# danielzgtg/TTS.cpp

Hardware: AMD Instinct MI355X
Metric: audio-sec/wall-sec (RTF^-1), Parler-TTS-mini v1 Q4_K AR decode + DAC decode (higher is better)
Workload: dtype q4_K weights x q8_K activations (int dot, f32 combine); DAC f16 im2col x f32 weights, f64 accumulate

## Files before the change

### include/tts_hip.h

```cpp
#ifndef TTS_HIP_H
#define TTS_HIP_H

#include <stddef.h>
#include <stdint.h>

#ifdef __cplusplus
extern "C" {
#endif

#define TTS_MAX_DIMS 4
#define TTS_MAX_SRC 4
#define TTS_MAX_OP_PARAMS 16
#define TTS_MAX_NAME 64

enum tts_type {
    TTS_TYPE_F32 = 0,
    TTS_TYPE_F16 = 1,
    TTS_TYPE_Q4_0 = 2,
    TTS_TYPE_Q4_1 = 3,
    TTS_TYPE_Q5_0 = 6,
    TTS_TYPE_Q5_1 = 7,
    TTS_TYPE_Q8_0 = 8,
    TTS_TYPE_Q8_1 = 9,
    TTS_TYPE_Q4_K = 12,
// ... 167 lines not shown
    TTS_HIP_OPT_GEMV_RSPLIT = 17,
    TTS_HIP_OPT_ATTN_PV16 = 15,
    TTS_HIP_OPT_GEMV_PREQUANT = 21,
    TTS_HIP_OPT_GEMV_KRELAY = 22,
    TTS_HIP_OPT_ATTN_KS = 23,
    TTS_HIP_OPT_ATTN_PV8 = 24,
    TTS_HIP_OPT_GEMV_KRELAY_LOOP = 26,
    TTS_HIP_OPT_GEMV_Q80_PRO = 27,
    TTS_HIP_OPT_GEMV_Q80_SLAB = 28,
    TTS_HIP_OPT_GEMV_Q80_RW = 29,
    TTS_HIP_OPT_GEMM_Q8_STAGED = 30,
    TTS_HIP_OPT_GEMV_KR_INKERNEL = 31,
    TTS_HIP_OPT_GEMV_F32_WIDE = 32,
    TTS_HIP_OPT_ATTN_PV_MP = 33,
    TTS_HIP_OPT_GEMM_KR_INKERNEL = 35,
    TTS_HIP_OPT_GEMM_KR_CT2 = 36,
    TTS_HIP_OPT_GEMM_KR_NW = 34,
    TTS_HIP_OPT_GEMV_NW_MIN = 25,
    TTS_HIP_OPT_GEMM_KR_XCD = 38,
    TTS_HIP_OPT_GEMM_KR_CP = 39,
    TTS_HIP_OPT_GEMM_KR_WALK = 40,
    TTS_HIP_OPT_GEMM_PF = 41,
    TTS_HIP_OPT_GEMM_PF_NW = 42,
    TTS_HIP_OPT_ATTN_ONE = 43,
    TTS_HIP_OPT_GEMV_KR_TAIL = 44,
    TTS_HIP_OPT_GEMV_Q50_SLAB = 45,
    TTS_HIP_OPT_GEMV_Q50_RW = 46,
    TTS_HIP_OPT_GEMM_Q5 = 47,
    TTS_HIP_OPT_GEMM_Q5_STAGED = 48,
    TTS_HIP_OPT_GEMV_Q40_SLAB = 49,
    TTS_HIP_OPT_GEMV_Q40_RW = 50,
    TTS_HIP_OPT_GEMM_Q4_0 = 51,
    TTS_HIP_OPT_GEMM_Q4_0_STAGED = 52,
    TTS_HIP_OPT_COALESCE = 37,
};
enum tts_fuse_bits {
    TTS_FUSE_LN = 1, TTS_FUSE_GROUP = 2, TTS_FUSE_KV = 4, TTS_FUSE_EPI = 8, TTS_FUSE_HEADS = 16, TTS_FUSE_ATTN = 32,
    TTS_FUSE_LSTM = 64,
    TTS_FUSE_SNAKE = 128,
    TTS_FUSE_EMBED = 256,
    TTS_FUSE_CONV = 512,
    TTS_FUSE_ADAIN = 1024,
    TTS_FUSE_XATTN = 2048,
    TTS_FUSE_MCPY = 4096,
    TTS_FUSE_CONTREAD = 8192
};
int tts_hip_set_option(tts_hip_backend_t backend, int option, int value);
int tts_hip_attn_decode(tts_hip_backend_t backend, const tts_tensor * q, const tts_tensor * k, const tts_tensor * v,
                        const float * mask, int64_t mbs, float scale, float * out, float * out2, const int64_t * koff,
                        const int64_t * voff, const int64_t * moff, const int32_t * pseq);
int tts_hip_coalesce_stats(int device, int64_t * out, int n);
void tts_hip_coalesce_set_wait(int us);
int tts_hip_coalesce_enable(int on);
#define TTS_HIP_HOOK_FAULT_WEIGHT_SET 1
int tts_hip_test_hook(int hook, int value);
int tts_hip_install_crash_handler(void);
int tts_hip_gemv_stats(tts_hip_backend_t backend, int type, double * ms, int64_t * launches, double * bytes, int reset);
int tts_hip_greedy_step(tts_hip_backend_t backend, const float * logits, int32_t B, int32_t NH, int32_t V, int32_t step,
                        int32_t bos, int32_t eos, int32_t * eos_seen, int32_t * hist, int32_t * next);
typedef struct tts_sampling {
    float temperature;
    float top_p;
    float repetition_penalty;
    int32_t top_k;
    int32_t do_sample;
    int32_t pad_;
// ... 48 lines not shown
```

### tts.cpp_amd/csrc/backend.hip

```cpp
#include <cmath>
#include <atomic>
#include <cstring>
#include <map>
#include <mutex>
#include <thread>

#include "hip_internal.h"
#include <hip/hip_ext.h>

#include <dlfcn.h>
#include <execinfo.h>
#include <fcntl.h>
#include <signal.h>
#include <unistd.h>

using namespace tts;


static void build_gelu_table(uint16_t * t) {
    const float GELU_COEF_A = 0.044715f;
    const float SQRT_2_OVER_PI = 0.79788456080286535587989211986876f;
    for (int i = 0; i < 65536; ++i) {
        const float x = fp16_to_fp32_host((uint16_t)i);
        const float g = 0.5f * x * (1.0f + tanhf(SQRT_2_OVER_PI * x * (1.0f + GELU_COEF_A * x * x)));
// ... 50 lines not shown
    if (hipGetDeviceCount(&n) != hipSuccess) return 0;
    return n;
}

tts_hip_backend_t tts_hip_backend_init(int device) {
    int n = tts_hip_device_count();
    if (device < 0 || device >= n) return nullptr;
    if (hipSetDevice(device) != hipSuccess) return nullptr;
    auto * be = new tts_hip_backend();
    be->device = device;
    TTS_HIP_CHECK(hipStreamCreateWithFlags(&be->stream, hipStreamNonBlocking));
    TTS_HIP_CHECK(hipStreamCreateWithFlags(&be->cap_stream, hipStreamNonBlocking));
    TTS_HIP_CHECK(hipStreamCreateWithFlags(&be->pf_stream, hipStreamNonBlocking));
    TTS_HIP_CHECK(hipEventCreateWithFlags(&be->co_ev, hipEventDisableTiming));
    TTS_HIP_CHECK(hipEventCreateWithFlags(&be->pf_fork, hipEventDisableTiming));
    TTS_HIP_CHECK(hipEventCreateWithFlags(&be->pf_join, hipEventDisableTiming));
    hipDeviceProp_t prop;
    TTS_HIP_CHECK(hipGetDeviceProperties(&prop, device));
    snprintf(be->name, sizeof(be->name), "HIP%d(%s)", device, prop.gcnArchName);
    be->cu_total = prop.multiProcessorCount > 0 ? prop.multiProcessorCount : 256;
    be->cus = be->cu_total;
    TTS_HIP_CHECK(hipMalloc((void **)&be->scratch, kScratchBytes));
    be->scratch_size = kScratchBytes;
    TTS_HIP_CHECK(hipMalloc((void **)&be->shadow, kShadowBytes));
    be->shadow_size = kShadowBytes;
    be->hoist_size = (size_t)8 << 20;
    TTS_HIP_CHECK(hipMalloc(&be->hoist, be->hoist_size));
    TTS_HIP_CHECK(hipMalloc((void **)&be->lstm_buf, kLstmFloats * sizeof(float)));
    TTS_HIP_CHECK(hipMalloc((void **)&be->attn_buf, kAttnFloats * sizeof(float)));
    be->attn_floats = kAttnFloats;
    TTS_HIP_CHECK(hipMalloc((void **)&be->vec_scratch, kVecScratchFloats * sizeof(float)));
    be->conv_stage_floats = (size_t)8 << 20;
    TTS_HIP_CHECK(hipMalloc((void **)&be->conv_stage, be->conv_stage_floats * sizeof(float)));
    be->conv_part_doubles = (size_t)8 << 20;
    TTS_HIP_CHECK(hipMalloc((void **)&be->conv_part, be->conv_part_doubles * sizeof(double)));
    be->lstm_floats = kLstmFloats;
    TTS_HIP_CHECK(hipMalloc((void **)&be->argmax_keys, kArgmaxRows * sizeof(unsigned long long)));
    TTS_HIP_CHECK(hipMalloc((void **)&be->argmax_counts, kArgmaxRows * sizeof(unsigned)));
    TTS_HIP_CHECK(hipMemset(be->argmax_keys, 0, kArgmaxRows * sizeof(unsigned long long)));
    TTS_HIP_CHECK(hipMemset(be->argmax_counts, 0, kArgmaxRows * sizeof(unsigned)));
    TTS_HIP_CHECK(hipHostMalloc((void **)&be->pin, kPinBytes, hipHostMallocDefault));
    be->pin_size = kPinBytes;
    for (auto & e : be->plan_ev) TTS_HIP_CHECK(hipEventCreateWithFlags(&e, hipEventDisableTiming));
    std::vector<uint16_t> tab(65536);
    build_gelu_table(tab.data());
    TTS_HIP_CHECK(hipMalloc((void **)&be->gelu_table, 65536 * sizeof(uint16_t)));
    TTS_HIP_CHECK(hipMemcpy(be->gelu_table, tab.data(), 65536 * sizeof(uint16_t), hipMemcpyHostToDevice));
    return be;
}

void tts_hip_backend_free(tts_hip_backend_t be) {
    if (!be) return;
    tts::coalesce_backend_gone(be);
    hipSetDevice(be->device);
    hipStreamSynchronize(be->stream);
    for (auto & p : be->ev_pending) {
        hipEventDestroy(p.first);
        hipEventDestroy(p.second);
    }
    for (auto e : be->ev_free) hipEventDestroy(e);
    for (auto & r : be->pin_pending) hipEventDestroy(r.ev);
    for (auto e : be->pin_events) hipEventDestroy(e);
    for (auto e : be->plan_ev) hipEventDestroy(e);
    hipHostFree(be->pin);
    if (be->rb_host) hipHostFree(be->rb_host);
    hipFree(be->scratch);
// ... 551 lines not shown
        case TTS_OP_IM2COL:
            return is_f32(n->src[1]) && n->op_params[6] == 0 && (n->type == TTS_TYPE_F16 || n->type == TTS_TYPE_F32);
        case TTS_OP_CONV_TRANSPOSE_1D:
            return is_f32(n->src[0]) && is_f32(n->src[1]) && n->op_params[4] >= 1;
        case TTS_OP_CUMSUM: case TTS_OP_UPSCALE: case TTS_OP_STFT: case TTS_OP_ISTFT: case TTS_OP_MAP_CUSTOM3: case TTS_OP_MAP_CUSTOM2:
            return tts::audio_op_supported(n);
        case TTS_OP_GET_ROWS:
            return n->src[1]->type == TTS_TYPE_I32 &&
                   (n->src[0]->type == TTS_TYPE_F32 || n->src[0]->type == TTS_TYPE_F16 || n->src[0]->type == TTS_TYPE_Q4_K ||
                    n->src[0]->type == TTS_TYPE_Q8_0 || n->src[0]->type == TTS_TYPE_Q5_0 || n->src[0]->type == TTS_TYPE_Q4_0);
        case TTS_OP_MUL_MAT: {
            const tts_tensor * a = n->src[0];
            const tts_tensor * b = n->src[1];
            if (!is_f32(b)) return 0;
            if (a->ne[0] != b->ne[0] || b->ne[2] % a->ne[2] || b->ne[3] % a->ne[3]) return 0;
            if (a->type == TTS_TYPE_F32 || a->type == TTS_TYPE_F16) return 1;
            if (a->type == TTS_TYPE_Q4_K) return a->ne[0] % 256 == 0;
            if (a->type == TTS_TYPE_Q8_0 || a->type == TTS_TYPE_Q5_0 || a->type == TTS_TYPE_Q4_0) return a->ne[0] % 32 == 0;
            return 0;
        }
        default:
            return 0;
    }
}

}

extern "C" int tts_hip_set_option(tts_hip_backend_t be, int option, int value) {
    if (!be) return TTS_STATUS_BAD_ARG;
    switch (option) {
        case TTS_HIP_OPT_FUSION: be->fusion = value; return 0;
        case TTS_HIP_OPT_CONVT_LDS: be->convt_lds = value != 0; return 0;
        case TTS_HIP_OPT_CONV_SPLIT: be->conv_split = value < 0 ? 1 : value; return 0;
        case TTS_HIP_OPT_PROFILE_GEMV: be->profile_gemv = value != 0; return 0;
        case TTS_HIP_OPT_GRAPHS: be->use_graphs = value != 0; return 0;
        case TTS_HIP_OPT_CONV_F32ACC:
            be->conv_f32acc = value == 1;
            be->conv_acc_mode = value == 2 ? 2 : 0;
            return 0;
        case TTS_HIP_OPT_ATTN_SPLIT: be->attn_split_minp = value; return 0;
        case TTS_HIP_OPT_ATTN_FUSED: be->attn_fused_minp = value; return 0;
        case TTS_HIP_OPT_ATTN_PV16: be->attn_pv_uv16 = value != 0; return 0;
        case TTS_HIP_OPT_KV_PREFETCH: be->kv_prefetch_minp = value; return 0;
        case TTS_HIP_OPT_Q4K_TILE_BYTES: be->q4k_tile_bytes = value; return 0;
        case TTS_HIP_OPT_Q4K_DUAL_BYTES: be->q4k_dual_bytes = value; return 0;
        case TTS_HIP_OPT_GEMV_RSPLIT: be->gemv_mf_rsplit = value != 0; return 0;
        case TTS_HIP_OPT_GEMV_PREQUANT: be->gemv_mf_prequant = value != 0; return 0;
        case TTS_HIP_OPT_GEMV_KRELAY: be->gemv_kr = value != 0; return 0;
        case TTS_HIP_OPT_GEMV_KRELAY_LOOP: be->gemv_kr_loop = value != 0; return 0;
        case TTS_HIP_OPT_GEMV_Q80_PRO: be->gemv_q80_pro = value != 0; return 0;
        case TTS_HIP_OPT_GEMV_Q80_SLAB: be->gemv_q80_slab = value != 0; return 0;
        case TTS_HIP_OPT_GEMV_KR_INKERNEL:
            if (value < 0) return TTS_STATUS_BAD_ARG;
            be->gemv_kr_ink = value;
            return 0;
        case TTS_HIP_OPT_GEMM_Q8_STAGED:
            if (value < 0 || value > 2) return TTS_STATUS_BAD_ARG;
            be->gemm_q8_staged = value;
            return 0;
        case TTS_HIP_OPT_GEMV_Q80_RW:
            if (value < 0 || value > 32 || (value & (value - 1))) return TTS_STATUS_BAD_ARG;
            be->gemv_q80_rw = value;
            return 0;
        case TTS_HIP_OPT_GEMV_Q50_SLAB: be->gemv_q50_slab = value != 0; return 0;
        case TTS_HIP_OPT_GEMV_Q50_RW:
            if (value < 0 || value > 32 || (value & (value - 1))) return TTS_STATUS_BAD_ARG;
// ... 167 lines not shown
```

### tts.cpp_amd/csrc/hip_internal.h

```cpp
#pragma once

#include <hip/hip_fp16.h>
#include <hip/hip_runtime.h>

#include <cstdio>
#include <cstdlib>
#include <atomic>
#include <deque>
#include <mutex>
#include <unordered_map>
#include <tuple>
#include <vector>

#include "common.h"

#define TTS_HIP_CHECK(expr)                                                                          \
    do {                                                                                             \
        hipError_t err_ = (expr);                                                                    \
        if (err_ != hipSuccess) {                                                                    \
            fprintf(stderr, "%s:%d: HIP error %s: %s\n", __FILE__, __LINE__, #expr, hipGetErrorString(err_)); \
            abort();                                                                                 \
        }                                                                                            \
    } while (0)

// ... 370 lines not shown
    int gemm_kr_ct2 = 0;
    int64_t gemm_kr_ink = 0;
    int gemv_nw_min = 0;
    int gemv_mf_rsplit = 1;
    int64_t q4k_dual_bytes = 1 << 20;
    void * sample_cand = nullptr;
    size_t sample_cand_size = 0;
    int kv_prefetch_minp = 0;
    int kv_prefetch_blocks = 128;
    hipStream_t pf_stream = nullptr;
    hipEvent_t pf_fork = nullptr, pf_join = nullptr;
    uint8_t * pin = nullptr;
    size_t pin_size = 0, pin_head = 0;
    struct PinRec {
        size_t off, size;
        hipEvent_t ev;
    };
    std::deque<PinRec> pin_pending;
    std::vector<hipEvent_t> pin_events;
    std::mutex pin_mu;
    hipEvent_t plan_ev[2] = {nullptr, nullptr};
    bool plan_ev_pending[2] = {false, false};
    float * lstm_buf = nullptr;
    float * conv_stage = nullptr;
    size_t conv_stage_floats = 0;
    float * vec_scratch = nullptr;
    size_t lstm_floats = 0;
    tts::ActQuant aq;
    int64_t graph_epoch = 0;
    uint16_t * gelu_table = nullptr;
    bool convt_lds = true;
    double * conv_part = nullptr;
    size_t conv_part_doubles = 0;
    int conv_split = 1;
    int fusion = 0x3FFF;
    bool profile_gemv = false;
    double gemv_ms[TTS_TYPE_COUNT] = {0};
    int64_t gemv_launches[TTS_TYPE_COUNT] = {0};
    double gemv_bytes[TTS_TYPE_COUNT] = {0};
    std::vector<std::pair<hipEvent_t, hipEvent_t>> ev_pending;
    std::vector<double> ev_bytes;
    std::vector<int> ev_type;
    std::vector<hipEvent_t> ev_free;
    char * repack_tmp = nullptr;
    size_t repack_tmp_size = 0;
    std::vector<char *> repack_retired;
    float * attn_stage = nullptr;
    size_t attn_stage_size = 0;
    bool use_graphs = false;
    static constexpr int N_GSIG = 4;
    uint64_t gsig[N_GSIG] = {};
    hipGraphExec_t gsig_exec[N_GSIG] = {};
    int gsig_next = 0;
    bool conv_f32acc = false;
    int conv_acc_mode = 0;
    hipStream_t cap_stream = nullptr;
    int64_t graph_updates = 0, graph_instantiations = 0;
    int64_t lstm_chains = 0, lstm_steps = 0;
    int64_t plan_wait_ns = 0;
    int64_t cap_plan_ns = 0, cap_launch_ns = 0, cap_update_ns = 0;
    hipGraphExec_t pexec[2] = {nullptr, nullptr};
    tts_tensor * const * plan_nodes[2] = {nullptr, nullptr};
    int plan_n[2] = {0, 0};
    bool plan_eager[2] = {true, true};
    bool plan_prepared[2] = {false, false};
    tts::BatchCtx * bat = nullptr;
// ... 139 lines not shown
```

### tts.cpp_amd/csrc/k_conv.hip

```cpp
#include "hip_internal.h"

namespace tts {

template <bool F16OUT>
__global__ void k_im2col(TD dst, TD x, int K, int s0, int p0, int d0, int64_t n) {
    const int64_t KW = dst.ne[0];
    const int64_t OL = dst.ne[1];
    const int64_t L = x.ne[0];
    for (int64_t e = (int64_t)blockIdx.x * blockDim.x + threadIdx.x; e < n; e += (int64_t)gridDim.x * blockDim.x) {
        const int64_t kk = e % KW;
        const int64_t ol = (e / KW) % OL;
        const int64_t nn = e / (KW * OL);
        const int64_t ic = kk / K, k = kk % K;
        const int64_t il = ol * s0 + k * d0 - p0;
        float v = 0.f;
        if (il >= 0 && il < L) v = *(const float *)(x.data + il * x.nb[0] + ic * x.nb[1] + nn * x.nb[2]);
        char * o = dst.data + kk * dst.nb[0] + ol * dst.nb[1] + nn * dst.nb[2];
        if (F16OUT) *(__half *)o = __float2half_rn(v);
        else *(float *)o = v;
    }
}

void launch_im2col(tts_hip_backend * be, const tts_tensor * node) {
    const tts_tensor * a = node->src[0];
// ... 186 lines not shown
    if (a->ne[2] * a->ne[3] != 1 || b->ne[2] * b->ne[3] != 1 || node->type != TTS_TYPE_F32) return false;
    const int64_t K = a->ne[0], M = a->ne[1], N = b->ne[1];
    const size_t bes = tts_type_size(b->type);
    if (K % 8 || a->nb[0] != 2 || b->nb[0] != bes || node->nb[0] != 4) return false;
    if (a->nb[1] % 16 || b->nb[1] % 16 || ((uintptr_t)a->data % 16) || ((uintptr_t)b->data % 16)) return false;
    dim3 grid((unsigned)((M + 63) / 64), (unsigned)((N + 63) / 64));
    if (!be->conv_f32acc) {
        const int nz = split_count(be, (int64_t)grid.x * grid.y, K, 256, M * N);
        const int64_t kps = nz > 1 ? (((K + nz - 1) / nz + 31) & ~(int64_t)31) : K;
        const int nzr = nz > 1 ? (int)((K + kps - 1) / kps) : 1;
        double * part = nzr > 1 ? be->conv_part : nullptr;
        grid.z = (unsigned)nzr;
        if (b->type == TTS_TYPE_F16)
            hipLaunchKernelGGL(k_gemm_f16_f64acc<true>, grid, dim3(256), 0, be->stream, (const __half *)a->data, (int64_t)(a->nb[1] / 2), b->data,
                               (int64_t)(b->nb[1] / 2), (float *)node->data, (int64_t)(node->nb[1] / 4), M, N, K, part, kps);
        else
            hipLaunchKernelGGL(k_gemm_f16_f64acc<false>, grid, dim3(256), 0, be->stream, (const __half *)a->data, (int64_t)(a->nb[1] / 2), b->data,
                               (int64_t)(b->nb[1] / 4), (float *)node->data, (int64_t)(node->nb[1] / 4), M, N, K, part, kps);
        TTS_HIP_CHECK(hipGetLastError());
        if (part) launch_split_reduce(be, nzr, M, N, (float *)node->data, (int64_t)(node->nb[1] / 4), nullptr, 0, nullptr, 0);
        return true;
    }
    if (b->type == TTS_TYPE_F16)
        hipLaunchKernelGGL(k_gemm_f16_mfma<true>, grid, dim3(256), 0, be->stream, (const __half *)a->data, (int64_t)(a->nb[1] / 2), b->data,
                           (int64_t)(b->nb[1] / 2), (float *)node->data, (int64_t)(node->nb[1] / 4), M, N, K);
    else
        hipLaunchKernelGGL(k_gemm_f16_mfma<false>, grid, dim3(256), 0, be->stream, (const __half *)a->data, (int64_t)(a->nb[1] / 2), b->data,
                           (int64_t)(b->nb[1] / 4), (float *)node->data, (int64_t)(node->nb[1] / 4), M, N, K);
    TTS_HIP_CHECK(hipGetLastError());
    return true;
}

typedef _Float16 h16x8_t __attribute__((ext_vector_type(8)));
template <bool W16, bool BIAS, bool RES, bool H32 = false>
__global__ __launch_bounds__(256) void k_conv1d_f64(Conv1dArgs a) {
    extern __shared__ float sm[];
    __shared__ int xoff[CONV1D_MAX_R];
    __shared__ int wofs[CONV1D_MAX_R];
    const int lane = threadIdx.x & 63, wave = threadIdx.x >> 6;
    const int c16 = lane & 15, kq = lane >> 4;
    const int64_t ol0 = (int64_t)blockIdx.x * 64;
    const int oc0 = blockIdx.y * 64;
    const int K = a.K, s = a.s, icc = a.icc, xw = a.xw, rs = a.rs;
    const int R = icc * K, Rp = (R + 31) & ~31;
    float * xs = sm;
    float * ws = sm + icc * xw + 1;
    const int zslot = icc * xw;
    for (int r = threadIdx.x; r < Rp; r += 256) {
        const int ic = r / K, k = r - ic * K;
        xoff[r] = r < R ? ic * xw + k * a.d : zslot;
        wofs[r] = r < R ? (int)(k * a.wk + ic * a.wic) : -1;
    }
    if (threadIdx.x == 0) xs[zslot] = 0.f;
    __syncthreads();
    const int wr0 = (wave >> 1) * 32, wc0 = (wave & 1) * 32;
    const bool wave_live = oc0 + wr0 < a.OC && ol0 + wc0 < a.OL;
    f64x4_t acc[2][2] = {};
    const int64_t base = ol0 * s - a.p;
    const int EX = icc * xw, EW = 64 * Rp;
    constexpr int esz = W16 ? 2 : 4;
    const uint32_t OOB = 0x80000000u;
    const auto xr = __builtin_amdgcn_make_buffer_rsrc(a.x.data, 0, a.x_bytes, 0x00020000);
    const auto wr = __builtin_amdgcn_make_buffer_rsrc(const_cast<void *>(a.w), 0, a.w_bytes, 0x00020000);
    uint32_t xrel[CONV1D_XN], wrel[CONV1D_WN];
    int xic[CONV1D_XN], wic[CONV1D_WN];
#pragma unroll
    for (int u = 0; u < CONV1D_XN; ++u) {
        const int e = (int)threadIdx.x + 256 * u;
        const int ic = e / xw, q = e - ic * xw;
        const int64_t pos = base + q;
        const bool ok = e < EX && pos >= 0 && pos < a.L;
        xrel[u] = ok ? (uint32_t)(pos * a.x.nb[0] + (int64_t)ic * a.x.nb[1]) : OOB;
        xic[u] = e < EX ? ic : -1;
    }
#pragma unroll
    for (int u = 0; u < CONV1D_WN; ++u) {
        const int e = (int)threadIdx.x + 256 * u;
        const int oc = e / Rp, r = e - oc * Rp;
        const int wo = e < EW ? wofs[r] : -1;
        const bool ok = wo >= 0 && oc0 + oc < a.OC;
        wrel[u] = ok ? (uint32_t)(((int64_t)(oc0 + oc) * a.woc + wo) * esz) : OOB;
        wic[u] = e < EW ? (r < R ? r / K : icc) : -1;
    }
    float xv[CONV1D_XN], wv[CONV1D_WN];
    auto fetch = [&](int ic0) {
        const int nic = min(icc, (int)(a.IC - ic0));
        const uint32_t xc = (uint32_t)((int64_t)ic0 * a.x.nb[1]);
        const uint32_t wc = (uint32_t)((int64_t)ic0 * a.wic * esz);
#pragma unroll
        for (int u = 0; u < CONV1D_XN; ++u) {
            const uint32_t off = (xrel[u] == OOB || xic[u] >= nic) ? OOB : xrel[u] + xc;
            xv[u] = __builtin_bit_cast(float, __builtin_amdgcn_raw_buffer_load_b32(xr, off, 0, 0));
        }
#pragma unroll
        for (int u = 0; u < CONV1D_WN; ++u) {
            const uint32_t off = (wrel[u] == OOB || wic[u] >= nic) ? OOB : wrel[u] + wc;
            if (W16) wv[u] = __half2float(__builtin_bit_cast(__half, __builtin_amdgcn_raw_buffer_load_b16(wr, off, 0, 0)));
            else wv[u] = __builtin_bit_cast(float, __builtin_amdgcn_raw_buffer_load_b32(wr, off, 0, 0));
        }
    };
    const int ic_lo = a.part ? (int)blockIdx.z * a.ic_per_split : 0;
    const int ic_hi = a.part ? (int)min((int64_t)(ic_lo + a.ic_per_split), a.IC) : (int)a.IC;
    fetch(ic_lo);
    for (int ic0 = ic_lo; ic0 < ic_hi; ic0 += icc) {
#pragma unroll
        for (int u = 0; u < CONV1D_XN; ++u)
            if (xic[u] >= 0) xs[(int)threadIdx.x + 256 * u] = __half2float(__float2half_rn(xv[u]));
#pragma unroll
        for (int u = 0; u < CONV1D_WN; ++u)
            if (wic[u] >= 0) {
                const int e = (int)threadIdx.x + 256 * u;
                const int oc = e / Rp;
                ws[oc * rs + (e - oc * Rp)] = W16 ? wv[u] : __half2float(__float2half_rn(wv[u]));
            }
        __syncthreads();
        if (ic0 + icc < ic_hi) fetch(ic0 + icc);
        if (!wave_live) {
            __syncthreads();
            continue;
        }
        if (H32) {
            for (int r0 = 0; r0 < Rp; r0 += 32) {
                int xo[8];
#pragma unroll
                for (int u = 0; u < 8; ++u) xo[u] = xoff[r0 + 8 * kq + u];
                h16x8_t A[2], B[2];
#pragma unroll
                for (int t = 0; t < 2; ++t)
#pragma unroll
                    for (int u = 0; u < 8; ++u) {
                        const bool z = xo[u] == zslot;
                        A[t][u] = (_Float16)ws[(wr0 + 16 * t + c16) * rs + r0 + 8 * kq + u];
                        B[t][u] = (_Float16)xs[z ? zslot : xo[u] + (wc0 + 16 * t + c16) * s];
                    }
#pragma unroll
                for (int ti = 0; ti < 2; ++ti)
#pragma unroll
                    for (int tj = 0; tj < 2; ++tj) {
                        const f32x4 pr = __builtin_amdgcn_mfma_f32_16x16x32_f16(A[ti], B[tj], f32x4{0.f, 0.f, 0.f, 0.f}, 0, 0, 0);
#pragma unroll
                        for (int e = 0; e < 4; ++e) acc[ti][tj][e] += (double)pr[e];
                    }
            }
        } else
        for (int r0 = 0; r0 < Rp; r0 += 32) {
            int xo[8];
#pragma unroll
            for (int u = 0; u < 8; ++u) xo[u] = xoff[r0 + 4 * u + kq];
            float af[8][2], bf[8][2];
#pragma unroll
            for (int u = 0; u < 8; ++u) {
                const int r = r0 + 4 * u + kq;
                const bool z = xo[u] == zslot;
#pragma unroll
                for (int t = 0; t < 2; ++t) {
                    af[u][t] = ws[(wr0 + 16 * t + c16) * rs + r];
                    bf[u][t] = xs[z ? zslot : xo[u] + (wc0 + 16 * t + c16) * s];
                }
            }
#pragma unroll
            for (int u = 0; u < 8; ++u)
#pragma unroll
                for (int ti = 0; ti < 2; ++ti)
#pragma unroll
                    for (int tj = 0; tj < 2; ++tj)
                        acc[ti][tj] = __builtin_amdgcn_mfma_f64_16x16x4f64((double)af[u][ti], (double)bf[u][tj], acc[ti][tj], 0, 0, 0);
        }
        __syncthreads();
    }
    if (a.part) {
#pragma unroll
        for (int tj = 0; tj < 2; ++tj) {
            const int64_t ol = ol0 + wc0 + 16 * tj + c16;
            if (ol >= a.OL) continue;
#pragma unroll
            for (int ti = 0; ti < 2; ++ti)
#pragma unroll
                for (int e = 0; e < 4; ++e) {
                    const int oc = oc0 + wr0 + 16 * ti + (H32 ? 4 * kq + e : kq + 4 * e);
                    if (oc < a.OC) a.part[((int64_t)blockIdx.z * a.OC + oc) * a.OL + ol] = acc[ti][tj][e];
                }
        }
        return;
    }
    float bv[2][4], rv[2][2][4];
#pragma unroll
    for (int ti = 0; ti < 2; ++ti)
#pragma unroll
        for (int e = 0; e < 4; ++e) {
            const int oc = min(oc0 + wr0 + 16 * ti + (H32 ? 4 * kq + e : kq + 4 * e), (int)a.OC - 1);
            bv[ti][e] = BIAS ? a.bias[(int64_t)oc * a.bcs] : 0.f;
#pragma unroll
            for (int tj = 0; tj < 2; ++tj) {
                const int64_t ol = min(ol0 + wc0 + 16 * tj + c16, a.OL - 1);
                rv[tj][ti][e] = RES ? a.res[ol + (int64_t)oc * a.rcs] : 0.f;
            }
        }
#pragma unroll
    for (int tj = 0; tj < 2; ++tj) {
        const int64_t ol = ol0 + wc0 + 16 * tj + c16;
        if (ol >= a.OL) continue;
#pragma unroll
        for (int ti = 0; ti < 2; ++ti)
#pragma unroll
            for (int e = 0; e < 4; ++e) {
                const int oc = oc0 + wr0 + 16 * ti + (H32 ? 4 * kq + e : kq + 4 * e);
                if (oc >= a.OC) continue;
                float v = (float)acc[ti][tj][e];
                if (BIAS) v = v + bv[ti][e];
                if (RES) v = rv[tj][ti][e] + v;
                a.y[ol + (int64_t)oc * a.ycs] = v;
            }
    }
}

bool conv1d_fused_ok(int64_t IC, int K, int s, int d, size_t * lds) {
    if (K < 1 || K > 64 || s < 1 || d < 1 || IC < 1) return false;
    const int xw = 63 * s + (K - 1) * d + 1;
    const int icc = conv1d_icc(IC, K, xw);
    if (icc < 1) return false;
    const int rs = ((icc * K + 31) & ~31) + 1;
    const size_t bytes = ((size_t)icc * xw + 1 + 64 * (size_t)rs) * 4;
    if (lds) *lds = bytes;
    return bytes <= 64 * 1024;
}

void launch_conv1d_fused(tts_hip_backend * be, Conv1dArgs a) {
    a.xw = 63 * a.s + (a.K - 1) * a.d + 1;
    a.icc = conv1d_icc(a.IC, a.K, a.xw);
    a.rs = ((a.icc * a.K + 31) & ~31) + 1;
    size_t lds = 0;
    if (!conv1d_fused_ok(a.IC, a.K, a.s, a.d, &lds)) {
        fprintf(stderr, "tts_hip: conv1d_fused shape unsupported\n");
        abort();
    }
    dim3 grid((unsigned)((a.OL + 63) / 64), (unsigned)((a.OC + 63) / 64));
    Conv1dArgs e = a;
    const int64_t nchunk = (a.IC + a.icc - 1) / a.icc;
    const int nz = be->conv_acc_mode == 2 ? 1 : split_count(be, (int64_t)grid.x * grid.y, nchunk, 2, a.OL * a.OC);
    if (nz > 1) {
        a.ic_per_split = (int)(((nchunk + nz - 1) / nz) * a.icc);
        grid.z = (unsigned)((a.IC + a.ic_per_split - 1) / a.ic_per_split);
        a.part = be->conv_part;
        a.bias = nullptr;
        a.res = nullptr;
    }
    const int sel = (a.w16 ? 4 : 0) | (a.bias ? 2 : 0) | (a.res ? 1 : 0);
    if (be->conv_acc_mode == 2) switch (sel) {
        case 0: hipLaunchKernelGGL((k_conv1d_f64<false, false, false, true>), grid, dim3(256), lds, be->stream, a); break;
        case 1: hipLaunchKernelGGL((k_conv1d_f64<false, false, true, true>), grid, dim3(256), lds, be->stream, a); break;
        case 2: hipLaunchKernelGGL((k_conv1d_f64<false, true, false, true>), grid, dim3(256), lds, be->stream, a); break;
        case 3: hipLaunchKernelGGL((k_conv1d_f64<false, true, true, true>), grid, dim3(256), lds, be->stream, a); break;
        case 4: hipLaunchKernelGGL((k_conv1d_f64<true, false, false, true>), grid, dim3(256), lds, be->stream, a); break;
        case 5: hipLaunchKernelGGL((k_conv1d_f64<true, false, true, true>), grid, dim3(256), lds, be->stream, a); break;
        case 6: hipLaunchKernelGGL((k_conv1d_f64<true, true, false, true>), grid, dim3(256), lds, be->stream, a); break;
        default: hipLaunchKernelGGL((k_conv1d_f64<true, true, true, true>), grid, dim3(256), lds, be->stream, a); break;
    }
    else switch (sel) {
        case 0: hipLaunchKernelGGL((k_conv1d_f64<false, false, false>), grid, dim3(256), lds, be->stream, a); break;
        case 1: hipLaunchKernelGGL((k_conv1d_f64<false, false, true>), grid, dim3(256), lds, be->stream, a); break;
        case 2: hipLaunchKernelGGL((k_conv1d_f64<false, true, false>), grid, dim3(256), lds, be->stream, a); break;
        case 3: hipLaunchKernelGGL((k_conv1d_f64<false, true, true>), grid, dim3(256), lds, be->stream, a); break;
        case 4: hipLaunchKernelGGL((k_conv1d_f64<true, false, false>), grid, dim3(256), lds, be->stream, a); break;
        case 5: hipLaunchKernelGGL((k_conv1d_f64<true, false, true>), grid, dim3(256), lds, be->stream, a); break;
        case 6: hipLaunchKernelGGL((k_conv1d_f64<true, true, false>), grid, dim3(256), lds, be->stream, a); break;
        default: hipLaunchKernelGGL((k_conv1d_f64<true, true, true>), grid, dim3(256), lds, be->stream, a); break;
    }
    TTS_HIP_CHECK(hipGetLastError());
    if (a.part) launch_split_reduce(be, (int)grid.z, a.OL, a.OC, e.y, e.ycs, e.bias, e.bcs, e.res, e.rcs);
    if (a.copy_dst)
        launch_copy_bytes(be, a.copy_dst, a.y, (size_t)a.OL * (size_t)a.OC * 4);
}

__global__ __launch_bounds__(256) void k_conv_transpose_1d(TD y, TD x, TD w, int s, int p, int d, int g) {
    const int64_t OL = y.ne[0];
    const int64_t o = (int64_t)blockIdx.x * blockDim.x + threadIdx.x;
    const int oc = blockIdx.y;
    if (o >= OL) return;
    const int K = (int)w.ne[0], OCg = (int)w.ne[1];
    const int64_t L = x.ne[0];
    const int IC = (int)x.ne[1], ICg = IC / g;
    const int grp = oc / OCg, ocl = oc % OCg;
    double acc = 0.0;
    const int64_t num0 = o + p;
    for (int k = (d == 1 ? (int)(num0 % s) : 0); k < K; k += (d == 1 ? s : 1)) {
        const int64_t num = num0 - (int64_t)k * d;
        if (num < 0) break;
        if (num % s) continue;
        const int64_t i = num / s;
        if (i >= L) continue;
        const char * xp = x.data + i * x.nb[0] + (int64_t)grp * ICg * x.nb[1];
        const char * wp = w.data + (int64_t)k * w.nb[0] + (int64_t)ocl * w.nb[1] + (int64_t)grp * ICg * w.nb[2];
        if (w.type == TTS_TYPE_F16) {
            for (int icl = 0; icl < ICg; ++icl)
                acc = __fma_rn((double)__half2float(__float2half_rn(*(const float *)(xp + icl * x.nb[1]))),
                               (double)__half2float(*(const __half *)(wp + icl * w.nb[2])), acc);
        } else {
            for (int icl = 0; icl < ICg; ++icl)
                acc = __fma_rn((double)*(const float *)(xp + icl * x.nb[1]), (double)*(const float *)(wp + icl * w.nb[2]), acc);
        }
// ... 206 lines not shown
```

### tts.cpp_amd/ttship/__init__.py

```python
import ctypes
import os
import pathlib

_HERE = pathlib.Path(__file__).resolve().parent
PKG_ROOT = _HERE.parent
REPO_ROOT = PKG_ROOT.parent
LIB_PATH = PKG_ROOT / "lib" / "libtts_hip.so"

F32, F16, Q4_0, Q5_0, Q8_0, Q4_K, Q8_K, I32 = 0, 1, 2, 6, 8, 12, 15, 26
PROF_ATTN = 39

OPS = ["NONE", "DUP", "ADD", "SUB", "MUL", "DIV", "SQR", "SQRT", "SIN", "COS", "SUM_ROWS", "REPEAT",
       "CONCAT", "NORM", "RMS_NORM", "MUL_MAT", "SCALE", "CPY", "CONT", "RESHAPE", "VIEW", "PERMUTE",
       "TRANSPOSE", "GET_ROWS", "SOFT_MAX", "ROPE", "CLAMP", "CONV_TRANSPOSE_1D", "IM2COL", "UPSCALE",
       "PAD", "LEAKY_RELU", "UNARY", "CUMSUM", "MOD", "ROUND", "STFT", "ISTFT", "MAP_CUSTOM3", "MAP_CUSTOM2"]
OP = {n: i for i, n in enumerate(OPS)}
FUSE = {"LN": 1, "GROUP": 2, "KV": 4, "EPI": 8, "HEADS": 16, "ATTN": 32, "LSTM": 64, "SNAKE": 128, "EMBED": 256, "CONV": 512, "ADAIN": 1024, "XATTN": 2048, "MCPY": 4096, "CONTREAD": 8192}
FUSE_ALL = sum(FUSE.values())
UNARY = {"ABS": 0, "NEG": 1, "TANH": 2, "RELU": 3, "SIGMOID": 4, "GELU": 5, "SILU": 6, "EXP": 7}

OPT = {"FUSION": 0, "PROFILE_GEMV": 1, "GRAPHS": 2, "CONV_F32ACC": 3, "CONVT_LDS": 4, "ATTN_SPLIT": 5, "KV_PREFETCH": 6, "KV_PREFETCH_BLOCKS": 7, "Q4K_TILE_BYTES": 8, "GEMV_DEBUG": 10, "GEMV_UNIQUE": 11, "CONV_SPLIT": 12, "GEMV_KS": 13, "ATTN_FUSED": 14, "ATTN_PV16": 15, "Q4K_DUAL_BYTES": 16, "GEMV_RSPLIT": 17, "GEMM_Q8": 18, "BGEMM_F32": 19, "CU_PARTITION": 20, "GEMV_PREQUANT": 21, "GEMV_KRELAY": 22, "ATTN_KS": 23, "ATTN_PV8": 24, "GEMV_NW_MIN": 25, "GEMV_KRELAY_LOOP": 26, "GEMV_Q80_PRO": 27, "GEMV_Q80_SLAB": 28, "GEMV_Q80_RW": 29, "GEMM_Q8_STAGED": 30, "GEMV_KR_INKERNEL": 31, "GEMV_F32_WIDE": 32, "ATTN_PV_MP": 33, "GEMM_KR_NW": 34, "GEMM_KR_INKERNEL": 35, "GEMM_KR_CT2": 36, "COALESCE": 37, "GEMM_KR_XCD": 38, "GEMM_KR_CP": 39, "GEMM_KR_WALK": 40, "GEMM_PF": 41, "GEMM_PF_NW": 42, "ATTN_ONE": 43, "GEMV_KR_TAIL": 44, "GEMV_Q50_SLAB": 45, "GEMV_Q50_RW": 46, "GEMM_Q5": 47, "GEMM_Q5_STAGED": 48, "GEMV_Q40_SLAB": 49, "GEMV_Q40_RW": 50, "GEMM_Q4_0": 51, "GEMM_Q4_0_STAGED": 52}
ATTN_SPLIT_DEFAULT = 128
ATTN_ONE_DEFAULT = 1
GEMV_KR_TAIL_DEFAULT = 1
ATTN_FUSED_ON = 128

TYPE_SIZE = {F32: 4, F16: 2, Q4_K: 144, Q8_0: 34, Q5_0: 22, Q4_0: 18, I32: 4}
BLCK_SIZE = {F32: 1, F16: 1, Q4_K: 256, Q8_0: 32, Q5_0: 32, Q4_0: 32, I32: 1}


class TtsTensor(ctypes.Structure):
    pass


TtsTensor._fields_ = [
    ("type", ctypes.c_int32),
    ("op", ctypes.c_int32),
    ("ne", ctypes.c_int64 * 4),
    ("nb", ctypes.c_uint64 * 4),
    ("op_params", ctypes.c_int32 * 16),
    ("src", ctypes.POINTER(TtsTensor) * 4),
    ("view_src", ctypes.POINTER(TtsTensor)),
    ("view_offs", ctypes.c_uint64),
    ("data", ctypes.c_void_p),
    ("flags", ctypes.c_int32),
    ("pad_", ctypes.c_int32),
    ("name", ctypes.c_char * 64),
]


class BackendIface(ctypes.Structure):
    _fields_ = [
        ("ctx", ctypes.c_void_p),
        ("name", ctypes.c_char_p),
# ... 1508 lines not shown
```

Measured before the change: 111.0.

## Add vector-FMA f64 conv path for small OC and 96-row MFMA tile

Adds a scalar f64 FMA conv1d kernel used by default when output channels are fewer than 8 (e.g. the final DAC projection), so MFMA tiles are not mostly wasted on padding. Parameterizes the MFMA conv kernel by row-tile count so layers whose OC is a multiple of 96 use 96-row tiles with a waves-per-EU hint. It also simplifies the index math with shifts and drops the per-element channel arrays. The 96 tile raises LDS and register use, which may lower occupancy, and the new FMA kernel reads doubles from LDS with possible bank pressure.

```diff
diff --git a/include/tts_hip.h b/include/tts_hip.h
--- a/include/tts_hip.h
+++ b/include/tts_hip.h
@@ -223,6 +223,8 @@
     TTS_HIP_OPT_GEMV_Q40_RW = 50,
     TTS_HIP_OPT_GEMM_Q4_0 = 51,
     TTS_HIP_OPT_GEMM_Q4_0_STAGED = 52,
+    TTS_HIP_OPT_CONV_VFMA = 53,
+    TTS_HIP_OPT_CONV_TILE96 = 54,
     TTS_HIP_OPT_COALESCE = 37,
 };
 enum tts_fuse_bits {
diff --git a/tts.cpp_amd/csrc/backend.hip b/tts.cpp_amd/csrc/backend.hip
--- a/tts.cpp_amd/csrc/backend.hip
+++ b/tts.cpp_amd/csrc/backend.hip
@@ -106,6 +106,8 @@
     TTS_HIP_CHECK(hipMalloc((void **)&be->vec_scratch, kVecScratchFloats * sizeof(float)));
     be->conv_stage_floats = (size_t)8 << 20;
     TTS_HIP_CHECK(hipMalloc((void **)&be->conv_stage, be->conv_stage_floats * sizeof(float)));
+    if (const char * e = getenv("TTS_HIP_OPT_CONV_VFMA"))
+        if (e[0] >= '0' && e[0] <= '2' && !e[1]) be->conv_vfma = e[0] - '0';
     be->conv_part_doubles = (size_t)8 << 20;
     TTS_HIP_CHECK(hipMalloc((void **)&be->conv_part, be->conv_part_doubles * sizeof(double)));
     be->lstm_floats = kLstmFloats;
@@ -723,6 +725,8 @@
         case TTS_HIP_OPT_FUSION: be->fusion = value; return 0;
         case TTS_HIP_OPT_CONVT_LDS: be->convt_lds = value != 0; return 0;
         case TTS_HIP_OPT_CONV_SPLIT: be->conv_split = value < 0 ? 1 : value; return 0;
+        case TTS_HIP_OPT_CONV_VFMA: be->conv_vfma = value < 0 || value > 2 ? 1 : value; return 0;
+        case TTS_HIP_OPT_CONV_TILE96: be->conv_tile96 = value != 0; return 0;
         case TTS_HIP_OPT_PROFILE_GEMV: be->profile_gemv = value != 0; return 0;
         case TTS_HIP_OPT_GRAPHS: be->use_graphs = value != 0; return 0;
         case TTS_HIP_OPT_CONV_F32ACC:
diff --git a/tts.cpp_amd/csrc/hip_internal.h b/tts.cpp_amd/csrc/hip_internal.h
--- a/tts.cpp_amd/csrc/hip_internal.h
+++ b/tts.cpp_amd/csrc/hip_internal.h
@@ -426,6 +426,8 @@
     bool convt_lds = true;
     double * conv_part = nullptr;
     size_t conv_part_doubles = 0;
+    int conv_vfma = 1;
+    int conv_tile96 = 1;
     int conv_split = 1;
     int fusion = 0x3FFF;
     bool profile_gemv = false;
diff --git a/tts.cpp_amd/csrc/k_conv.hip b/tts.cpp_amd/csrc/k_conv.hip
--- a/tts.cpp_amd/csrc/k_conv.hip
+++ b/tts.cpp_amd/csrc/k_conv.hip
@@ -242,15 +242,25 @@
 }
 
 typedef _Float16 h16x8_t __attribute__((ext_vector_type(8)));
-template <bool W16, bool BIAS, bool RES, bool H32 = false>
-__global__ __launch_bounds__(256) void k_conv1d_f64(Conv1dArgs a) {
+
+template <bool BIAS, bool RES>
+__device__ __forceinline__ float conv1d_epilogue(double acc, float bias, float res) {
+    float v = (float)acc;
+    if (BIAS) v = v + bias;
+    if (RES) v = res + v;
+    return v;
+}
+
+template <bool W16, bool BIAS, bool RES, bool H32 = false, int MT = 2>
+__global__ __launch_bounds__(256) __attribute__((amdgpu_waves_per_eu(MT == 2 ? 1 : 2))) void k_conv1d_f64(Conv1dArgs a) {
+    constexpr int OCT = 32 * MT, WN = CONV1D_WN * MT / 2;
     extern __shared__ float sm[];
     __shared__ int xoff[CONV1D_MAX_R];
     __shared__ int wofs[CONV1D_MAX_R];
     const int lane = threadIdx.x & 63, wave = threadIdx.x >> 6;
     const int c16 = lane & 15, kq = lane >> 4;
     const int64_t ol0 = (int64_t)blockIdx.x * 64;
-    const int oc0 = blockIdx.y * 64;
+    const int oc0 = blockIdx.y * OCT;
     const int K = a.K, s = a.s, icc = a.icc, xw = a.xw, rs = a.rs;
     const int R = icc * K, Rp = (R + 31) & ~31;
     float * xs = sm;
@@ -263,17 +273,17 @@
     }
     if (threadIdx.x == 0) xs[zslot] = 0.f;
     __syncthreads();
-    const int wr0 = (wave >> 1) * 32, wc0 = (wave & 1) * 32;
+    const int wr0 = (wave >> 1) * 16 * MT, wc0 = (wave & 1) * 32;
     const bool wave_live = oc0 + wr0 < a.OC && ol0 + wc0 < a.OL;
-    f64x4_t acc[2][2] = {};
+    f64x4_t acc[MT][2] = {};
     const int64_t base = ol0 * s - a.p;
-    const int EX = icc * xw, EW = 64 * Rp;
+    const int EX = icc * xw, EW = OCT * Rp;
     constexpr int esz = W16 ? 2 : 4;
     const uint32_t OOB = 0x80000000u;
     const auto xr = __builtin_amdgcn_make_buffer_rsrc(a.x.data, 0, a.x_bytes, 0x00020000);
     const auto wr = __builtin_amdgcn_make_buffer_rsrc(const_cast<void *>(a.w), 0, a.w_bytes, 0x00020000);
-    uint32_t xrel[CONV1D_XN], wrel[CONV1D_WN];
-    int xic[CONV1D_XN], wic[CONV1D_WN];
+    const int rsh = Rp == 64 ? 6 : 5;
+    uint32_t xrel[CONV1D_XN], wrel[WN];
 #pragma unroll
     for (int u = 0; u < CONV1D_XN; ++u) {
         const int e = (int)threadIdx.x + 256 * u;
@@ -281,30 +291,28 @@
         const int64_t pos = base + q;
         const bool ok = e < EX && pos >= 0 && pos < a.L;
         xrel[u] = ok ? (uint32_t)(pos * a.x.nb[0] + (int64_t)ic * a.x.nb[1]) : OOB;
-        xic[u] = e < EX ? ic : -1;
-    }
-#pragma unroll
-    for (int u = 0; u < CONV1D_WN; ++u) {
+    }
+#pragma unroll
+    for (int u = 0; u < WN; ++u) {
         const int e = (int)threadIdx.x + 256 * u;
-        const int oc = e / Rp, r = e - oc * Rp;
+        const int oc = e >> rsh, r = e & (Rp - 1);
         const int wo = e < EW ? wofs[r] : -1;
         const bool ok = wo >= 0 && oc0 + oc < a.OC;
         wrel[u] = ok ? (uint32_t)(((int64_t)(oc0 + oc) * a.woc + wo) * esz) : OOB;
-        wic[u] = e < EW ? (r < R ? r / K : icc) : -1;
-    }
-    float xv[CONV1D_XN], wv[CONV1D_WN];
+    }
+    float xv[CONV1D_XN], wv[WN];
     auto fetch = [&](int ic0) {
         const int nic = min(icc, (int)(a.IC - ic0));
         const uint32_t xc = (uint32_t)((int64_t)ic0 * a.x.nb[1]);
         const uint32_t wc = (uint32_t)((int64_t)ic0 * a.wic * esz);
 #pragma unroll
         for (int u = 0; u < CONV1D_XN; ++u) {
-            const uint32_t off = (xrel[u] == OOB || xic[u] >= nic) ? OOB : xrel[u] + xc;
+            const uint32_t off = (xrel[u] == OOB || (int)threadIdx.x + 256 * u >= nic * xw) ? OOB : xrel[u] + xc;
             xv[u] = __builtin_bit_cast(float, __builtin_amdgcn_raw_buffer_load_b32(xr, off, 0, 0));
         }
 #pragma unroll
-        for (int u = 0; u < CONV1D_WN; ++u) {
-            const uint32_t off = (wrel[u] == OOB || wic[u] >= nic) ? OOB : wrel[u] + wc;
+        for (int u = 0; u < WN; ++u) {
+            const uint32_t off = (wrel[u] == OOB || (((int)threadIdx.x + 256 * u) & (Rp - 1)) >= nic * K) ? OOB : wrel[u] + wc;
             if (W16) wv[u] = __half2float(__builtin_bit_cast(__half, __builtin_amdgcn_raw_buffer_load_b16(wr, off, 0, 0)));
             else wv[u] = __builtin_bit_cast(float, __builtin_amdgcn_raw_buffer_load_b32(wr, off, 0, 0));
         }
@@ -315,14 +323,12 @@
     for (int ic0 = ic_lo; ic0 < ic_hi; ic0 += icc) {
 #pragma unroll
         for (int u = 0; u < CONV1D_XN; ++u)
-            if (xic[u] >= 0) xs[(int)threadIdx.x + 256 * u] = __half2float(__float2half_rn(xv[u]));
-#pragma unroll
-        for (int u = 0; u < CONV1D_WN; ++u)
-            if (wic[u] >= 0) {
-                const int e = (int)threadIdx.x + 256 * u;
-                const int oc = e / Rp;
-                ws[oc * rs + (e - oc * Rp)] = W16 ? wv[u] : __half2float(__float2half_rn(wv[u]));
-            }
+            if ((int)threadIdx.x + 256 * u < EX) xs[(int)threadIdx.x + 256 * u] = __half2float(__float2half_rn(xv[u]));
+#pragma unroll
+        for (int u = 0; u < WN; ++u) {
+            const int e = (int)threadIdx.x + 256 * u;
+            if (e < EW) ws[e + (e >> rsh)] = W16 ? wv[u] : __half2float(__float2half_rn(wv[u]));
+        }
         __syncthreads();
         if (ic0 + icc < ic_hi) fetch(ic0 + icc);
         if (!wave_live) {
@@ -334,17 +340,17 @@
                 int xo[8];
 #pragma unroll
                 for (int u = 0; u < 8; ++u) xo[u] = xoff[r0 + 8 * kq + u];
-                h16x8_t A[2], B[2];
-#pragma unroll
-                for (int t = 0; t < 2; ++t)
-#pragma unroll
-                    for (int u = 0; u < 8; ++u) {
-                        const bool z = xo[u] == zslot;
-                        A[t][u] = (_Float16)ws[(wr0 + 16 * t + c16) * rs + r0 + 8 * kq + u];
-                        B[t][u] = (_Float16)xs[z ? zslot : xo[u] + (wc0 + 16 * t + c16) * s];
-                    }
-#pragma unroll
-                for (int ti = 0; ti < 2; ++ti)
+                h16x8_t A[MT], B[2];
+#pragma unroll
+                for (int u = 0; u < 8; ++u) {
+                    const bool z = xo[u] == zslot;
+#pragma unroll
+                    for (int t = 0; t < MT; ++t) A[t][u] = (_Float16)ws[(wr0 + 16 * t + c16) * rs + r0 + 8 * kq + u];
+#pragma unroll
+                    for (int t = 0; t < 2; ++t) B[t][u] = (_Float16)xs[z ? zslot : xo[u] + (wc0 + 16 * t + c16) * s];
+                }
+#pragma unroll
+                for (int ti = 0; ti < MT; ++ti)
 #pragma unroll
                     for (int tj = 0; tj < 2; ++tj) {
                         const f32x4 pr = __builtin_amdgcn_mfma_f32_16x16x32_f16(A[ti], B[tj], f32x4{0.f, 0.f, 0.f, 0.f}, 0, 0, 0);
@@ -357,21 +363,20 @@
             int xo[8];
 #pragma unroll
             for (int u = 0; u < 8; ++u) xo[u] = xoff[r0 + 4 * u + kq];
-            float af[8][2], bf[8][2];
+            float af[8][MT], bf[8][2];
 #pragma unroll
             for (int u = 0; u < 8; ++u) {
                 const int r = r0 + 4 * u + kq;
                 const bool z = xo[u] == zslot;
 #pragma unroll
-                for (int t = 0; t < 2; ++t) {
-                    af[u][t] = ws[(wr0 + 16 * t + c16) * rs + r];
-                    bf[u][t] = xs[z ? zslot : xo[u] + (wc0 + 16 * t + c16) * s];
-                }
+                for (int t = 0; t < MT; ++t) af[u][t] = ws[(wr0 + 16 * t + c16) * rs + r];
+#pragma unroll
+                for (int t = 0; t < 2; ++t) bf[u][t] = xs[z ? zslot : xo[u] + (wc0 + 16 * t + c16) * s];
             }
 #pragma unroll
             for (int u = 0; u < 8; ++u)
 #pragma unroll
-                for (int ti = 0; ti < 2; ++ti)
+                for (int ti = 0; ti < MT; ++ti)
 #pragma unroll
                     for (int tj = 0; tj < 2; ++tj)
                         acc[ti][tj] = __builtin_amdgcn_mfma_f64_16x16x4f64((double)af[u][ti], (double)bf[u][tj], acc[ti][tj], 0, 0, 0);
@@ -384,7 +389,7 @@
             const int64_t ol = ol0 + wc0 + 16 * tj + c16;
             if (ol >= a.OL) continue;
 #pragma unroll
-            for (int ti = 0; ti < 2; ++ti)
+            for (int ti = 0; ti < MT; ++ti)
 #pragma unroll
                 for (int e = 0; e < 4; ++e) {
                     const int oc = oc0 + wr0 + 16 * ti + (H32 ? 4 * kq + e : kq + 4 * e);
@@ -393,9 +398,9 @@
         }
         return;
     }
-    float bv[2][4], rv[2][2][4];
-#pragma unroll
-    for (int ti = 0; ti < 2; ++ti)
+    float bv[MT][4], rv[2][MT][4];
+#pragma unroll
+    for (int ti = 0; ti < MT; ++ti)
 #pragma unroll
         for (int e = 0; e < 4; ++e) {
             const int oc = min(oc0 + wr0 + 16 * ti + (H32 ? 4 * kq + e : kq + 4 * e), (int)a.OC - 1);
@@ -411,17 +416,97 @@
         const int64_t ol = ol0 + wc0 + 16 * tj + c16;
         if (ol >= a.OL) continue;
 #pragma unroll
-        for (int ti = 0; ti < 2; ++ti)
+        for (int ti = 0; ti < MT; ++ti)
 #pragma unroll
             for (int e = 0; e < 4; ++e) {
                 const int oc = oc0 + wr0 + 16 * ti + (H32 ? 4 * kq + e : kq + 4 * e);
                 if (oc >= a.OC) continue;
-                float v = (float)acc[ti][tj][e];
-                if (BIAS) v = v + bv[ti][e];
-                if (RES) v = rv[tj][ti][e] + v;
-                a.y[ol + (int64_t)oc * a.ycs] = v;
-            }
-    }
+                a.y[ol + (int64_t)oc * a.ycs] = conv1d_epilogue<BIAS, RES>(acc[ti][tj][e], bv[ti][e], rv[tj][ti][e]);
+            }
+    }
+}
+
+constexpr int CONV1DV_NP = 4;
+template <bool W16, bool BIAS, bool RES>
+__global__ __launch_bounds__(256) void k_conv1d_f64v(Conv1dArgs a) {
+    constexpr int NP = CONV1DV_NP;
+    extern __shared__ double smd[];
+    const int K = a.K, d = a.d, icc = a.icc, xw = a.xw, R = icc * K;
+    double * xs = smd;
+    double * ws = smd + icc * xw;
+    const int tid = threadIdx.x;
+    const int64_t ol0 = (int64_t)blockIdx.x * (256 * NP);
+    const int oc = blockIdx.y;
+    const int64_t base = ol0 - a.p;
+    const int EX = icc * xw;
+    constexpr int esz = W16 ? 2 : 4;
+    const uint32_t OOB = 0x80000000u;
+    const auto xr = __builtin_amdgcn_make_buffer_rsrc(a.x.data, 0, a.x_bytes, 0x00020000);
+    const auto wr = __builtin_amdgcn_make_buffer_rsrc(const_cast<void *>(a.w), 0, a.w_bytes, 0x00020000);
+    uint32_t xrel[CONV1D_XN];
+#pragma unroll
+    for (int u = 0; u < CONV1D_XN; ++u) {
+        const int e = tid + 256 * u;
+        const int ic = e / xw, q = e - ic * xw;
+        const int64_t pos = base + q;
+        const bool ok = e < EX && pos >= 0 && pos < a.L;
+        xrel[u] = ok ? (uint32_t)(pos * a.x.nb[0] + (int64_t)ic * a.x.nb[1]) : OOB;
+    }
+    const int wicl = tid < R ? tid / K : -1;
+    const uint32_t wrel = tid < R ? (uint32_t)(((int64_t)oc * a.woc + (int64_t)(tid - wicl * K) * a.wk + (int64_t)wicl * a.wic) * esz) : OOB;
+    float xv[CONV1D_XN], wv;
+    auto fetch = [&](int ic0) {
+        const int nic = min(icc, (int)(a.IC - ic0));
+        const uint32_t xc = (uint32_t)((int64_t)ic0 * a.x.nb[1]);
+        const uint32_t wc = (uint32_t)((int64_t)ic0 * a.wic * esz);
+#pragma unroll
+        for (int u = 0; u < CONV1D_XN; ++u) {
+            const uint32_t off = (xrel[u] == OOB || tid + 256 * u >= nic * xw) ? OOB : xrel[u] + xc;
+            xv[u] = __builtin_bit_cast(float, __builtin_amdgcn_raw_buffer_load_b32(xr, off, 0, 0));
+        }
+        const uint32_t off = (wrel == OOB || wicl >= nic) ? OOB : wrel + wc;
+        if (W16) wv = __half2float(__builtin_bit_cast(__half, __builtin_amdgcn_raw_buffer_load_b16(wr, off, 0, 0)));
+        else wv = __builtin_bit_cast(float, __builtin_amdgcn_raw_buffer_load_b32(wr, off, 0, 0));
+    };
+    double acc[NP];
+#pragma unroll
+    for (int j = 0; j < NP; ++j) acc[j] = 0.0;
+    fetch(0);
+    for (int ic0 = 0; ic0 < a.IC; ic0 += icc) {
+        const int nic = min(icc, (int)(a.IC - ic0));
+#pragma unroll
+        for (int u = 0; u < CONV1D_XN; ++u)
+            if (tid + 256 * u < EX) xs[tid + 256 * u] = (double)__half2float(__float2half_rn(xv[u]));
+        if (wicl >= 0) ws[tid] = (double)(W16 ? wv : __half2float(__float2half_rn(wv)));
+        __syncthreads();
+        if (ic0 + icc < a.IC) fetch(ic0 + icc);
+        const double * xp = xs + tid;
+        for (int icl = 0; icl < nic; ++icl, xp += xw)
+            for (int k = 0; k < K; ++k) {
+                const double w = ws[icl * K + k];
+#pragma unroll
+                for (int j = 0; j < NP; ++j) acc[j] = __builtin_fma(xp[k * d + 256 * j], w, acc[j]);
+            }
+        __syncthreads();
+    }
+    const float bias = BIAS ? a.bias[(int64_t)oc * a.bcs] : 0.f;
+#pragma unroll
+    for (int j = 0; j < NP; ++j) {
+        const int64_t ol = ol0 + tid + 256 * j;
+        if (ol >= a.OL) continue;
+        const float res = RES ? a.res[ol + (int64_t)oc * a.rcs] : 0.f;
+        a.y[ol + (int64_t)oc * a.ycs] = conv1d_epilogue<BIAS, RES>(acc[j], bias, res);
+    }
+}
+
+static bool conv1d_vfma_geometry(const Conv1dArgs & a, int * xw, int * icc, size_t * lds) {
+    if (a.s != 1 || a.K < 1 || a.K > 64 || a.OC > 65535) return false;
+    const int64_t w = 256 * CONV1DV_NP + (int64_t)(a.K - 1) * a.d;
+    if (w > 256 * CONV1D_XN) return false;
+    int c = (int)std::min<int64_t>(std::min<int64_t>(a.IC, 256 * CONV1D_XN / w), 256 / a.K);
+    if (c < 1) return false;
+    *xw = (int)w, *icc = c, *lds = ((size_t)c * (size_t)w + (size_t)c * a.K) * sizeof(double);
+    return true;
 }
 
 bool conv1d_fused_ok(int64_t IC, int K, int s, int d, size_t * lds) {
@@ -456,26 +541,35 @@
         a.res = nullptr;
     }
     const int sel = (a.w16 ? 4 : 0) | (a.bias ? 2 : 0) | (a.res ? 1 : 0);
-    if (be->conv_acc_mode == 2) switch (sel) {
-        case 0: hipLaunchKernelGGL((k_conv1d_f64<false, false, false, true>), grid, dim3(256), lds, be->stream, a); break;
-        case 1: hipLaunchKernelGGL((k_conv1d_f64<false, false, true, true>), grid, dim3(256), lds, be->stream, a); break;
-        case 2: hipLaunchKernelGGL((k_conv1d_f64<false, true, false, true>), grid, dim3(256), lds, be->stream, a); break;
-        case 3: hipLaunchKernelGGL((k_conv1d_f64<false, true, true, true>), grid, dim3(256), lds, be->stream, a); break;
-        case 4: hipLaunchKernelGGL((k_conv1d_f64<true, false, false, true>), grid, dim3(256), lds, be->stream, a); break;
-        case 5: hipLaunchKernelGGL((k_conv1d_f64<true, false, true, true>), grid, dim3(256), lds, be->stream, a); break;
-        case 6: hipLaunchKernelGGL((k_conv1d_f64<true, true, false, true>), grid, dim3(256), lds, be->stream, a); break;
-        default: hipLaunchKernelGGL((k_conv1d_f64<true, true, true, true>), grid, dim3(256), lds, be->stream, a); break;
-    }
-    else switch (sel) {
-        case 0: hipLaunchKernelGGL((k_conv1d_f64<false, false, false>), grid, dim3(256), lds, be->stream, a); break;
-        case 1: hipLaunchKernelGGL((k_conv1d_f64<false, false, true>), grid, dim3(256), lds, be->stream, a); break;
-        case 2: hipLaunchKernelGGL((k_conv1d_f64<false, true, false>), grid, dim3(256), lds, be->stream, a); break;
-        case 3: hipLaunchKernelGGL((k_conv1d_f64<false, true, true>), grid, dim3(256), lds, be->stream, a); break;
-        case 4: hipLaunchKernelGGL((k_conv1d_f64<true, false, false>), grid, dim3(256), lds, be->stream, a); break;
-        case 5: hipLaunchKernelGGL((k_conv1d_f64<true, false, true>), grid, dim3(256), lds, be->stream, a); break;
-        case 6: hipLaunchKernelGGL((k_conv1d_f64<true, true, false>), grid, dim3(256), lds, be->stream, a); break;
-        default: hipLaunchKernelGGL((k_conv1d_f64<true, true, true>), grid, dim3(256), lds, be->stream, a); break;
-    }
+#define TTS_CONV1D_SEL(KERNEL, GRID, LDS, ...)                                                                           \
+    switch (sel) {                                                                                                        \
+        case 0: hipLaunchKernelGGL((KERNEL<false, false, false __VA_ARGS__>), GRID, dim3(256), LDS, be->stream, a); break; \
+        case 1: hipLaunchKernelGGL((KERNEL<false, false, true __VA_ARGS__>), GRID, dim3(256), LDS, be->stream, a); break;  \
+        case 2: hipLaunchKernelGGL((KERNEL<false, true, false __VA_ARGS__>), GRID, dim3(256), LDS, be->stream, a); break;  \
+        case 3: hipLaunchKernelGGL((KERNEL<false, true, true __VA_ARGS__>), GRID, dim3(256), LDS, be->stream, a); break;   \
+        case 4: hipLaunchKernelGGL((KERNEL<true, false, false __VA_ARGS__>), GRID, dim3(256), LDS, be->stream, a); break;  \
+        case 5: hipLaunchKernelGGL((KERNEL<true, false, true __VA_ARGS__>), GRID, dim3(256), LDS, be->stream, a); break;   \
+        case 6: hipLaunchKernelGGL((KERNEL<true, true, false __VA_ARGS__>), GRID, dim3(256), LDS, be->stream, a); break;   \
+        default: hipLaunchKernelGGL((KERNEL<true, true, true __VA_ARGS__>), GRID, dim3(256), LDS, be->stream, a); break;   \
+    }
+#define TTS_COMMA ,
+    int vxw = 0, vicc = 0;
+    size_t vlds = 0;
+    if (nz == 1 && be->conv_acc_mode != 2 && be->conv_vfma && (be->conv_vfma == 2 || a.OC < 8) && conv1d_vfma_geometry(a, &vxw, &vicc, &vlds)) {
+        a.xw = vxw, a.icc = vicc;
+        const dim3 vgrid((unsigned)((a.OL + 256 * CONV1DV_NP - 1) / (256 * CONV1DV_NP)), (unsigned)a.OC);
+        TTS_CONV1D_SEL(k_conv1d_f64v, vgrid, vlds)
+    } else if (nz == 1 && be->conv_acc_mode != 2 && be->conv_tile96 && a.OC % 96 == 0) {
+        grid.y = (unsigned)(a.OC / 96);
+        lds += 32 * (size_t)a.rs * 4;
+        TTS_CONV1D_SEL(k_conv1d_f64, grid, lds, TTS_COMMA false TTS_COMMA 3)
+    } else if (be->conv_acc_mode == 2) {
+        TTS_CONV1D_SEL(k_conv1d_f64, grid, lds, TTS_COMMA true)
+    } else {
+        TTS_CONV1D_SEL(k_conv1d_f64, grid, lds)
+    }
+#undef TTS_COMMA
+#undef TTS_CONV1D_SEL
     TTS_HIP_CHECK(hipGetLastError());
     if (a.part) launch_split_reduce(be, (int)grid.z, a.OL, a.OC, e.y, e.ycs, e.bias, e.bcs, e.res, e.rcs);
     if (a.copy_dst)
diff --git a/tts.cpp_amd/ttship/__init__.py b/tts.cpp_amd/ttship/__init__.py
--- a/tts.cpp_amd/ttship/__init__.py
+++ b/tts.cpp_amd/ttship/__init__.py
@@ -19,7 +19,7 @@
 FUSE_ALL = sum(FUSE.values())
 UNARY = {"ABS": 0, "NEG": 1, "TANH": 2, "RELU": 3, "SIGMOID": 4, "GELU": 5, "SILU": 6, "EXP": 7}
 
-OPT = {"FUSION": 0, "PROFILE_GEMV": 1, "GRAPHS": 2, "CONV_F32ACC": 3, "CONVT_LDS": 4, "ATTN_SPLIT": 5, "KV_PREFETCH": 6, "KV_PREFETCH_BLOCKS": 7, "Q4K_TILE_BYTES": 8, "GEMV_DEBUG": 10, "GEMV_UNIQUE": 11, "CONV_SPLIT": 12, "GEMV_KS": 13, "ATTN_FUSED": 14, "ATTN_PV16": 15, "Q4K_DUAL_BYTES": 16, "GEMV_RSPLIT": 17, "GEMM_Q8": 18, "BGEMM_F32": 19, "CU_PARTITION": 20, "GEMV_PREQUANT": 21, "GEMV_KRELAY": 22, "ATTN_KS": 23, "ATTN_PV8": 24, "GEMV_NW_MIN": 25, "GEMV_KRELAY_LOOP": 26, "GEMV_Q80_PRO": 27, "GEMV_Q80_SLAB": 28, "GEMV_Q80_RW": 29, "GEMM_Q8_STAGED": 30, "GEMV_KR_INKERNEL": 31, "GEMV_F32_WIDE": 32, "ATTN_PV_MP": 33, "GEMM_KR_NW": 34, "GEMM_KR_INKERNEL": 35, "GEMM_KR_CT2": 36, "COALESCE": 37, "GEMM_KR_XCD": 38, "GEMM_KR_CP": 39, "GEMM_KR_WALK": 40, "GEMM_PF": 41, "GEMM_PF_NW": 42, "ATTN_ONE": 43, "GEMV_KR_TAIL": 44, "GEMV_Q50_SLAB": 45, "GEMV_Q50_RW": 46, "GEMM_Q5": 47, "GEMM_Q5_STAGED": 48, "GEMV_Q40_SLAB": 49, "GEMV_Q40_RW": 50, "GEMM_Q4_0": 51, "GEMM_Q4_0_STAGED": 52}
+OPT = {"FUSION": 0, "PROFILE_GEMV": 1, "GRAPHS": 2, "CONV_F32ACC": 3, "CONVT_LDS": 4, "ATTN_SPLIT": 5, "KV_PREFETCH": 6, "KV_PREFETCH_BLOCKS": 7, "Q4K_TILE_BYTES": 8, "GEMV_DEBUG": 10, "GEMV_UNIQUE": 11, "CONV_SPLIT": 12, "GEMV_KS": 13, "ATTN_FUSED": 14, "ATTN_PV16": 15, "Q4K_DUAL_BYTES": 16, "GEMV_RSPLIT": 17, "GEMM_Q8": 18, "BGEMM_F32": 19, "CU_PARTITION": 20, "GEMV_PREQUANT": 21, "GEMV_KRELAY": 22, "ATTN_KS": 23, "ATTN_PV8": 24, "GEMV_NW_MIN": 25, "GEMV_KRELAY_LOOP": 26, "GEMV_Q80_PRO": 27, "GEMV_Q80_SLAB": 28, "GEMV_Q80_RW": 29, "GEMM_Q8_STAGED": 30, "GEMV_KR_INKERNEL": 31, "GEMV_F32_WIDE": 32, "ATTN_PV_MP": 33, "GEMM_KR_NW": 34, "GEMM_KR_INKERNEL": 35, "GEMM_KR_CT2": 36, "COALESCE": 37, "GEMM_KR_XCD": 38, "GEMM_KR_CP": 39, "GEMM_KR_WALK": 40, "GEMM_PF": 41, "GEMM_PF_NW": 42, "ATTN_ONE": 43, "GEMV_KR_TAIL": 44, "GEMV_Q50_SLAB": 45, "GEMV_Q50_RW": 46, "GEMM_Q5": 47, "GEMM_Q5_STAGED": 48, "GEMV_Q40_SLAB": 49, "GEMV_Q40_RW": 50, "GEMM_Q4_0": 51, "GEMM_Q4_0_STAGED": 52, "CONV_VFMA": 53, "CONV_TILE96": 54}
 ATTN_SPLIT_DEFAULT = 128
 ATTN_ONE_DEFAULT = 1
 GEMV_KR_TAIL_DEFAULT = 1
```

Result: faster. 114.9, median of 6 (+3.6%).
